# kvcache-ai/ktransformers

Measured on NVIDIA H100. Metric: decode tok/s DeepSeek-V3 671B INT4 (Q4_K_M) MoE-block hot path; HBM GB/s vs roofline, higher is better.
Workload: dtype int8xint4/int6->int32 dp4a, fp32 scales+accumulate, bf16 in/out

## Files before the change

### ktransformers_b200/csrc/handles.cuh

```cuda
#pragma once
#include "common.cuh"

namespace ktb {
enum FmtId { FMT_Q4K, FMT_Q5K, FMT_Q6K8, FMT_Q6K4T, FMT_GENK, FMT_RAWINT4, FMT_NONE };
enum Q6Layout { LAYOUT_RAW = 0, LAYOUT_SOA8 = 1, LAYOUT_T4 = 2 };

static inline FmtId pick_fmt(int type, int layout) {
    if (type == KTB200_TYPE_Q4_K) return FMT_Q4K;
    if (type == KTB200_TYPE_Q5_K) return FMT_Q5K;
    if (type == KTB200_TYPE_Q6_K && layout == LAYOUT_SOA8) return FMT_Q6K8;
    if (type == KTB200_TYPE_Q6_K && layout == LAYOUT_T4) return FMT_Q6K4T;
    if (is_kquant(type) || is_iquant(type)) return FMT_GENK;
    if (is_rawint4(type)) return FMT_RAWINT4;
    return FMT_NONE;
}
}

struct ktb200_mlp {
    int H, I, gate_type, up_type, down_type, hidden_type, group_max_len, device;
    const void *gate, *up, *down;
    bool loaded, gu_soa;
    int down_layout;
    float* inter;
};
// ... 1 lines not shown
struct ktb200_moe {
    ktb200_moe_config cfg;
    int device;
    bool loaded;
    bool gu_soa;
    int down_layout;
    float* inter;
    int64_t* ids_d;
    float* w_d;
    void* in_d;
    void* out_d;
    float* blk_partial;
    unsigned* blk_sync;
    unsigned blk_flip;
    float* blk_inter;
    uint8_t* blk_stage;
    const void* pf[3];
    size_t pf_bytes[3];
};

namespace ktb {
constexpr int kBlockMaxTokens = 8;
constexpr int kBlkStatusWord = 4, kBlkReadyWord = 8;
static inline size_t blk_ready_words(const ktb200_moe_config& c) {
    const int t = c.group_max_len < kBlockMaxTokens ? c.group_max_len : kBlockMaxTokens;
    return (size_t)t * (c.routed_expert_num + 1) * (c.intermediate_size / QK_K);
}
}

struct DeviceGuard {
    int prev;
    bool ok;
    explicit DeviceGuard(int dev) : prev(0), ok(true) {
        if (cudaGetDevice(&prev) != cudaSuccess) ok = false;
        if (ok && prev != dev && cudaSetDevice(dev) != cudaSuccess) ok = false;
    }
    ~DeviceGuard() { cudaSetDevice(prev); }
};
```

### ktransformers_b200/csrc/moe.cu

```cuda
#include <cstdio>
#include <cstdlib>
#include <cstring>
#include <new>

#define KTB_IQ_CODEBOOKS
#include "gemv_bulk.cuh"
#include "dense_bulk.cuh"
#include "rawint4.cuh"
#include "iq.cuh"
#include "handles.cuh"

namespace ktb {

__global__ void __launch_bounds__(256) repack_q6k_kernel(uint8_t* w, long n_groups, int nb) {
    extern __shared__ __align__(16) uint8_t smem[];
    const long gbytes = 8L * SZ_Q6_K * nb;
    for (long g = blockIdx.x; g < n_groups; g += gridDim.x) {
        uint8_t* base = w + g * gbytes;
        for (long i = threadIdx.x; i < gbytes / 16; i += blockDim.x)
            reinterpret_cast<uint4*>(smem)[i] = reinterpret_cast<const uint4*>(base)[i];
        __syncthreads();
        const uint16_t* src = reinterpret_cast<const uint16_t*>(smem);
        uint16_t* dst = reinterpret_cast<uint16_t*>(base);
        const long s_qh = 1024L * nb, s_sc = 1536L * nb, s_d = 1664L * nb;
// ... 559 lines not shown
        set_error("MOEConfig: hidden_size %d and intermediate_size %d must be multiples of 256 for K-quant tensors",
                  c->hidden_size, c->intermediate_size);
        return KTB200_EINVAL;
    }
    if (!c->gate_proj || !c->up_proj || !c->down_proj) { set_error("MOEConfig: null weight pointer"); return KTB200_EINVAL; }
    DeviceGuard g(device);
    if (!g.ok) { set_error("cudaSetDevice(%d) failed", device); return KTB200_ECUDA; }
    ktb200_moe* m = new (std::nothrow) ktb200_moe();
    if (!m) return KTB200_ENOMEM;
    m->cfg = *c;
    m->device = device;
    m->loaded = false;
    m->gu_soa = false;
    m->down_layout = LAYOUT_RAW;
    m->inter = nullptr; m->ids_d = nullptr; m->w_d = nullptr; m->in_d = nullptr; m->out_d = nullptr;
    m->blk_partial = nullptr; m->blk_sync = nullptr; m->blk_flip = 0; m->blk_inter = nullptr; m->blk_stage = nullptr;
    for (int r = 0; r < 3; r++) { m->pf[r] = nullptr; m->pf_bytes[r] = 0; }
    const size_t slots = (size_t)c->group_max_len * c->routed_expert_num;
    const size_t hid = (size_t)c->group_max_len * c->hidden_size * type_size(c->hidden_type);
    cudaError_t e = cudaMalloc(&m->inter, (slots + c->group_max_len) * c->intermediate_size * sizeof(float));
    if (e == cudaSuccess) e = cudaMalloc(&m->ids_d, slots * sizeof(int64_t));
    if (e == cudaSuccess) e = cudaMalloc(&m->w_d, slots * sizeof(float));
    if (e == cudaSuccess) e = cudaMalloc(&m->in_d, hid);
    if (e == cudaSuccess) e = cudaMalloc(&m->out_d, hid);
    if (e == cudaSuccess) e = cudaMalloc(&m->blk_partial, (size_t)8 * 8 * 512 * sizeof(float));
    const size_t sync_words = kBlkReadyWord + 2 * blk_ready_words(*c);
    if (e == cudaSuccess) e = cudaMalloc(&m->blk_sync, sync_words * sizeof(unsigned));
    if (e == cudaSuccess) e = cudaMemset(m->blk_sync, 0, sync_words * sizeof(unsigned));
    if (e == cudaSuccess) e = cudaMalloc(&m->blk_inter, blk_ready_words(*c) * QK_K * sizeof(float));
    if (e == cudaSuccess) e = cudaMemset(m->blk_inter, 0xff, blk_ready_words(*c) * QK_K * sizeof(float));
    if (e == cudaSuccess) e = cudaMalloc(&m->blk_stage, blk_ready_words(*c) * (QK_K + 32 + 4));
    if (e != cudaSuccess) {
        set_error("cudaMalloc failed: %s", cudaGetErrorString(e));
        ktb200_moe_destroy(m);
        return KTB200_ENOMEM;
    }
    *out = m;
    return KTB200_OK;
}

void ktb200_moe_destroy(ktb200_moe* m) {
    if (!m) return;
    DeviceGuard g(m->device);
    cudaFree(m->inter); cudaFree(m->ids_d); cudaFree(m->w_d); cudaFree(m->in_d); cudaFree(m->out_d);
    cudaFree(m->blk_partial); cudaFree(m->blk_sync); cudaFree(m->blk_inter); cudaFree(m->blk_stage);
    delete m;
}

int ktb200_moe_load_weights(ktb200_moe* m, void* stream) {
    if (!m) { set_error("null handle"); return KTB200_EINVAL; }
    if (m->loaded) return KTB200_OK;
    DeviceGuard g(m->device);
    const ktb200_moe_config& c = m->cfg;
    cudaStream_t s = (cudaStream_t)stream;
    if (c.gate_type == KTB200_TYPE_Q6_K && c.up_type == KTB200_TYPE_Q6_K && c.intermediate_size % 8 == 0) {
        int rc = repack_q6k(const_cast<void*>(c.gate_proj), (long)c.expert_num * c.intermediate_size, c.hidden_size, m->device, s);
        if (rc) return rc;
        rc = repack_q6k(const_cast<void*>(c.up_proj), (long)c.expert_num * c.intermediate_size, c.hidden_size, m->device, s);
        if (rc) return rc;
        m->gu_soa = true;
// ... 341 lines not shown
```

### ktransformers_b200/csrc/moe_block.cu

```cuda
#include <cstdlib>

#include "gate.cuh"
#include "gemv_bulk.cuh"
#include "handles.cuh"

namespace ktb {

constexpr int kBlockWarps = 15;
constexpr int kBlockWarpsLo = 12;

struct BlockParams {
    GateParams g;
    const void *w_gate, *w_up, *w_down;
    const void *s_gate, *s_up, *s_down;
    int n_local, id_offset;
    int H, I, k;
    int hidden_type, use_silu;
    float* inter;
    void* out;
    unsigned* sync;
    unsigned* ready;
    unsigned* status;
    uint8_t* stage_q;
    int16_t* stage_bs;
    float* stage_d;
    int nrows_max;
    int region_a;
    int ring_bytes;
    int prime_u, prime_d;
    unsigned long long* trace;
    const uint8_t* pf[3];
    unsigned pf_bytes[3];
};

__device__ __forceinline__ unsigned ld_acquire_u32(const unsigned* p) {
    unsigned v;
    asm volatile("ld.acquire.gpu.global.u32 %0, [%1];" : "=r"(v) : "l"(p) : "memory");
    return v;
}
__device__ __forceinline__ unsigned ld_acquire_sys_u32(const unsigned* p) {
// ... 31 lines not shown
__device__ __forceinline__ void grid_wait(unsigned* counter, unsigned gen) {
    if (threadIdx.x == 0) {
        const unsigned target = gen * gridDim.x;
        while (ld_acquire_u32(counter) < target) {}
    }
    __syncthreads();
}


__device__ __forceinline__ void trace_stamp(const BlockParams& p, int i) {
    if (p.trace) p.trace[blockIdx.x * 16 + i] = ep_now();
}
__device__ __forceinline__ void block_stamp(const BlockParams& p, int i) {
    if (threadIdx.x == 0) trace_stamp(p, i);
}

__device__ __forceinline__ float4 load_x4(const void* x, long i4, int type) {
    if (type == KTB200_TYPE_F32) return reinterpret_cast<const float4*>(x)[i4];
    const uint2 v = reinterpret_cast<const uint2*>(x)[i4];
    if (type == KTB200_TYPE_BF16)
        return make_float4(__uint_as_float(v.x << 16), __uint_as_float(v.x & 0xffff0000u), __uint_as_float(v.y << 16),
                           __uint_as_float(v.y & 0xffff0000u));
    const float2 a = __half22float2(*reinterpret_cast<const __half2*>(&v.x)), b = __half22float2(*reinterpret_cast<const __half2*>(&v.y));
    return make_float4(a.x, a.y, b.x, b.y);
}

struct BlockShared {
    BlockParams prm;
    int64_t ids[32];
    float w[32];
    int vs[36];
    int nv;
    unsigned skip;
    int ent_state[36];
    int last_cta;
};
constexpr int kBlockSharedBytes = (sizeof(BlockShared) + 15) & ~15;

struct BlockLay {
    uint8_t *xq, *aq;
    int16_t *xbs, *abs_;
    float *xdx, *adx, *sel, *partial;
    size_t ring_off;
};
template <int KBS>
__device__ __forceinline__ BlockLay block_layout(const BlockParams& p, uint8_t* smem) {
    const int nblk = p.H / QK_K, nb = p.I / QK_K, ns = p.k + (p.s_gate ? 1 : 0);
    uint8_t* a = smem + kBlockSharedBytes;
    BlockLay L;
// ... 87 lines not shown
        int nv = p.s_gate ? 1 : 0;
        for (int j = 0; j < k; j++) {
            const long e = (long)sh.ids[j] - p.id_offset;
            if (e < 0 || e >= p.n_local) sk |= 1u << j; else sh.vs[nv++] = j;
        }
        sh.nv = nv;
        sh.skip = sk;
    }
    if (blockIdx.x == 0 && threadIdx.x < k) {
        p.g.idx[(long)t * k + threadIdx.x] = sh.ids[threadIdx.x];
        p.g.w[(long)t * k + threadIdx.x] = sh.w[threadIdx.x];
    }
    __syncthreads();
}

__device__ __forceinline__ void entry_slice(int I, int ie, int& r0, int& len) {
    const unsigned s = (blockIdx.x + (unsigned)ie) % gridDim.x;
    r0 = (int)((unsigned long long)I * s / gridDim.x);
    len = (int)((unsigned long long)I * (s + 1) / gridDim.x) - r0;
}

constexpr unsigned kInterEmpty = 0xffffffffu;
__device__ __forceinline__ void st_relaxed_f32(float* p, float v) {
    asm volatile("st.relaxed.gpu.global.f32 [%0], %1;" ::"l"(p), "f"(v) : "memory");
}
__device__ __forceinline__ uint4 ld_relaxed_u4(const void* p) {
    uint4 v;
    asm volatile("ld.relaxed.gpu.global.v4.u32 {%0, %1, %2, %3}, [%4];" : "=r"(v.x), "=r"(v.y), "=r"(v.z), "=r"(v.w) : "l"(p) : "memory");
    return v;
}

template <int KBS>
__device__ __forceinline__ void quantise_block(const BlockParams& p, long gb, float* src) {
    const int lane = threadIdx.x & 31;
    uint4 v0, v1;
    unsigned long long t0 = 0;
    for (unsigned spins = 1;; spins++) {
        v0 = ld_relaxed_u4(src + lane * 8);
        v1 = ld_relaxed_u4(src + lane * 8 + 4);
        const bool here = v0.x != kInterEmpty && v0.y != kInterEmpty && v0.z != kInterEmpty && v0.w != kInterEmpty &&
                          v1.x != kInterEmpty && v1.y != kInterEmpty && v1.z != kInterEmpty && v1.w != kInterEmpty;
        if (__all_sync(0xffffffffu, here)) break;
        if ((spins & 255u) == 0) {
            const unsigned long long t = ep_now();
            if (!t0) t0 = t;
            else if (t - t0 > kEpTimeoutNs) { if (lane == 0) *p.status = 1; break; }
        }
    }
    const float x[8] = {__uint_as_float(v0.x), __uint_as_float(v0.y), __uint_as_float(v0.z), __uint_as_float(v0.w),
                        __uint_as_float(v1.x), __uint_as_float(v1.y), __uint_as_float(v1.z), __uint_as_float(v1.w)};
    warp_quantize_q8k_block(x, lane, reinterpret_cast<uint32_t*>(p.stage_q + gb * QK_K), p.stage_d + gb,
                            KBS == 16 ? p.stage_bs + gb * 16 : nullptr, KBS == 8 ? p.stage_bs + gb * 8 : nullptr);
    const uint4 empty = make_uint4(kInterEmpty, kInterEmpty, kInterEmpty, kInterEmpty);
    reinterpret_cast<uint4*>(src + lane * 8)[0] = empty;
    reinterpret_cast<uint4*>(src + lane * 8)[1] = empty;
    __syncwarp();
    if (lane == 0) {
        __threadfence();
        atomicExch(p.ready + gb, 2u);
    }
}

template <int KBS>
__device__ __forceinline__ void claim_entry(const BlockParams& p, int t, int slot) {
    const int lane = threadIdx.x & 31, ns = p.k + (p.s_gate ? 1 : 0), nb = p.I / QK_K;
    const long g0 = ((long)t * ns + slot) * nb;
    for (int c0 = 0; c0 < nb; c0 += 32) {
        const int nc = min(32, nb - c0), rot = (int)(blockIdx.x % nc);
        for (;;) {
            const unsigned fr = __ballot_sync(0xffffffffu, lane < nc && ld_acquire_u32(p.ready + g0 + c0 + lane) == 0u);
            if (!fr) break;
            const unsigned pref = fr & (~0u << rot);
            const int b = c0 + __ffs(pref ? pref : fr) - 1;
            unsigned won = 0;
            if (lane == 0) won = atomicCAS(p.ready + g0 + b, 0u, 1u) == 0u;
            if (__shfl_sync(0xffffffffu, won, 0)) quantise_block<KBS>(p, g0 + b, p.inter + ((long)t * ns + slot) * p.I + (long)b * QK_K);
        }
    }
}

template <int KBS>
__device__ __forceinline__ void entry_to_smem(BlockShared& sh, const BlockLay& L, int t, int ev, bool need) {
    const BlockParams& p = sh.prm;
    const int lane = threadIdx.x & 31;
    volatile int* state = &sh.ent_state[ev];
    int s = lane == 0 ? *state : 0;
    s = __shfl_sync(0xffffffffu, s, 0);
    if (s == 0) {
        if (lane == 0) s = atomicCAS(&sh.ent_state[ev], 0, 1) == 0 ? 3 : 1;
        s = __shfl_sync(0xffffffffu, s, 0);
    }
    if (s == 3) {
        const int nb = p.I / QK_K, slot = sh.vs[ev];
        const long g0 = ((long)t * (p.k + (p.s_gate ? 1 : 0)) + slot) * nb;
        for (int b = lane; b < nb; b += 32) wait_ge<false>(p.ready + g0 + b, 2u, p.status);
        __syncwarp();
        const uint4* q = reinterpret_cast<const uint4*>(p.stage_q + g0 * QK_K);
        for (int i = lane; i < nb * (QK_K / 16); i += 32)
            *reinterpret_cast<uint4*>(L.aq + (size_t)(slot * nb + i / (QK_K / 16)) * kActBlkStride + (i % (QK_K / 16)) * 16) = __ldcg(q + i);
        const uint4* bs = reinterpret_cast<const uint4*>(p.stage_bs + g0 * KBS);
        for (int i = lane; i < nb * KBS / 8; i += 32) reinterpret_cast<uint4*>(L.abs_ + slot * nb * KBS)[i] = __ldcg(bs + i);
        for (int i = lane; i < nb; i += 32) L.adx[slot * nb + i] = __ldcg(p.stage_d + g0 + i);
        __syncwarp();
        if (lane == 0) {
            __threadfence_block();
            *state = 2;
            if (ev == 0) trace_stamp(p, 6);
            if (ev == sh.nv - 1) trace_stamp(p, 7);
        }
    } else if (s == 1 && need && lane == 0) {
        while (*state != 2) {}
    }
    if (lane == 0) __threadfence_block();
    __syncwarp();
}

template <int KBS>
__device__ __forceinline__ void blk_combine(int t) {
    extern __shared__ __align__(16) uint8_t smem[];
    const BlockShared& sh = *reinterpret_cast<const BlockShared*>(smem);
    const BlockParams& p = sh.prm;
    const BlockLay L = block_layout<KBS>(p, smem);
    const int k = p.k, ns = k + (p.s_gate ? 1 : 0);
    const int quads = p.H / 4;
    const int q0 = (int)((long)quads * blockIdx.x / gridDim.x), nrows = ((int)((long)quads * (blockIdx.x + 1) / gridDim.x) - q0) * 4;
    const unsigned skip = sh.skip;
// ... 30 lines not shown
    if (lane == 0) {
#pragma unroll
        for (int s = 0; s < SU; s++) mbar_init(bar_u32 + 8 * s, 1);
        mbar_fence_init();
        fence_proxy_async_smem();
    }
    {
        const uint32_t* src = reinterpret_cast<const uint32_t*>(&p);
        uint32_t* dst = reinterpret_cast<uint32_t*>(&sh.prm);
        for (int i = threadIdx.x; i < (int)(sizeof(BlockParams) / 4); i += blockDim.x) dst[i] = src[i];
    }
    if (threadIdx.x == 0 && has_shared) sh.vs[0] = k;
    uint32_t phase = 0;
    unsigned gen = 0;
    block_stamp(p, 0);

  for (int t = 0; t < Teff; t++) {
    __syncthreads();
    {
        const int nblk = p.H / QK_K, row_bytes = nblk * SZ_Q4_K;
        const int ns = k + (has_shared ? 1 : 0);
        int ie = 0, ir = 0, ir0 = 0, ilen = 0, ileft = 0, isub = 0;
        int ce = 0, cr = 0, cr0 = 0, clen = 0, cleft = 0, csub = 0;
        int stride = W, iend = 1;
        int slot_i = 0, slot_u = 0;
        auto advance = [&](int& e, int& r, int& r0, int& len, int n) {
            int off = r - r0 + n;
            while (off >= len && e + 1 < iend) { off -= len; e++; entry_slice(p.I, e, r0, len); }
            r = r0 + off;
        };
        auto start_list = [&](int e0, int e1, int first, int count, int stride_) {
            iend = e1;
            ie = e0;
            entry_slice(p.I, e0, ir0, ilen);
            ir = ir0;
            advance(ie, ir, ir0, ilen, first);
            ce = ie; cr = ir; cr0 = ir0; clen = ilen;
            ileft = cleft = count > 0 ? count : 0;
            stride = stride_;
        };
        auto issue_u = [&]() {
            if (ileft > 0 && isub - csub < SU) {
                if (lane == 0) {
                    const int s = sh.vs[ie];
                    const bool second = isub & 1;
                    const uint8_t* src;
                    if (s == k) {
                        src = reinterpret_cast<const uint8_t*>(second ? p.s_up : p.s_gate) + (long)ir * row_bytes;
                    } else {
                        const long e = (long)sh.ids[s] - p.id_offset;
                        src = reinterpret_cast<const uint8_t*>(second ? p.w_up : p.w_gate) + (e * p.I + ir) * row_bytes;
                    }
                    const uint32_t bar = bar_u32 + 8 * slot_i;
                    mbar_expect_tx(bar, (uint32_t)row_bytes);
                    bulk_g2s(ring_u32 + slot_i * row_bytes, src, (uint32_t)row_bytes, bar);
                }
                isub++;
                if (!(isub & 1)) {
                    ileft--;
                    advance(ie, ir, ir0, ilen, stride);
                }
                slot_i = (slot_i + 1 == SU) ? 0 : slot_i + 1;
            }
        };
        if (threadIdx.x < 36) sh.ent_state[threadIdx.x] = 0;
        blk_router(t, waited);
        block_stamp(p, 2);
        grid_arrive(p.sync, gen);
        if (has_shared && warp >= kGateWarps) {
            int r0, nr;
            entry_slice(p.I, 0, r0, nr);
            const int first = warp - kGateWarps, st = W - kGateWarps;
            start_list(0, 1, first, (nr - first + st - 1) / st, st);
        }
#pragma unroll
        for (int s = 0; s < SU; s++)
            if (s < p.prime_u) issue_u();
        blk_quantize_x(t);
        block_stamp(p, 1);
        grid_wait(p.sync, gen);
        block_stamp(p, 3);
        const BlockLay L = block_layout<DownFmt::kBs>(p, smem);
        const uint8_t* ring = smem + (ring_u32 - (uint32_t)__cvta_generic_to_shared(smem));
#pragma unroll 1
        for (int list = 0; list < 2; list++) {
            if (list == 1) {
                blk_select(t);
                block_stamp(p, 4);
                const int e0 = has_shared ? 1 : 0, nv = sh.nv;
                int total = 0;
                for (int e = e0; e < nv; e++) {
                    int r0, len;
                    entry_slice(p.I, e, r0, len);
                    total += len;
                }
                start_list(e0, nv, warp, (total - warp + W - 1) / W, W);
#pragma unroll
                for (int s = 0; s < SU; s++) issue_u();
            }
            float acc_first = 0.f;
            while (cleft > 0) {
                mbar_wait(bar_u32 + 8 * slot_u, (phase >> slot_u) & 1u);
                phase ^= 1u << slot_u;
                const uint8_t* row0 = ring + slot_u * row_bytes;
                float acc = 0.f;
                if (lane < nblk)
                    acc = q4k_block_dot(row0 + lane * SZ_Q4_K, L.xq + (size_t)lane * kActBlkStride,
                                        *reinterpret_cast<const uint4*>(L.xbs + lane * 8), L.xdx[lane]);
                __syncwarp();
                slot_u = (slot_u + 1 == SU) ? 0 : slot_u + 1;
                csub++;
                issue_u();
                if (csub & 1) { acc_first = acc; continue; }
                float g = acc_first, uu = acc;
#pragma unroll
                for (int o = 16; o > 0; o >>= 1) {
                    g += __shfl_xor_sync(0xffffffffu, g, o);
                    uu += __shfl_xor_sync(0xffffffffu, uu, o);
                }
                if (lane == 0) st_relaxed_f32(p.inter + ((long)t * ns + sh.vs[ce]) * p.I + cr, (p.use_silu ? act_silu(g) : act_relu(g)) * uu);
                cleft--;
                advance(ce, cr, cr0, clen, stride);
            }
        }
        __syncthreads();
        block_stamp(p, 5);
    }
    {
        const int nb = p.I / QK_K, nrb = RW * nb, item_bytes = nrb * DownFmt::kBlockBytes;
        const int quads = p.H / RW;
        const int q0 = (int)((long)quads * blockIdx.x / gridDim.x), nquads = (int)((long)quads * (blockIdx.x + 1) / gridDim.x) - q0;
        const int nv = sh.nv;
        const int Wd = W - 1;
        int ni = warp < Wd ? nquads * nv - warp : 0;
        ni = ni > 0 ? (ni + Wd - 1) / Wd : 0;
        int dvi = 0, dq = 0, dss = 0, dcons = 0;
        if (ni > 0) { dvi = warp / nquads; dq = warp - dvi * nquads; }
        int evi = dvi, eq = dq;
        int dslot_i = 0, dslot_u = 0;
        auto issue_d = [&]() {
            if (dss < ni && dss - dcons < SD) {
                if (lane == 0) {
                    const int j = sh.vs[dvi];
                    long row = (long)(q0 + dq) * RW;
                    const uint8_t* wbase = reinterpret_cast<const uint8_t*>(p.w_down);
                    if (j == k) wbase = reinterpret_cast<const uint8_t*>(p.s_down);
                    else row += ((long)sh.ids[j] - p.id_offset) * p.H;
                    const uint32_t bar = bar_u32 + 8 * dslot_i;
                    mbar_expect_tx(bar, (uint32_t)item_bytes);
                    bulk_g2s(ring_u32 + dslot_i * item_bytes, wbase + (row >> 2) * item_bytes, (uint32_t)item_bytes, bar);
                }
                dss++;
                dq += Wd;
                while (dq >= nquads) { dq -= nquads; dvi++; }
                dslot_i = (dslot_i + 1 == SD) ? 0 : dslot_i + 1;
            }
        };
#pragma unroll
        for (int s = 0; s < SD; s++) issue_d();
        const BlockLay L = block_layout<DownFmt::kBs>(p, smem);
        if (warp == W - 1) {
            for (int ev = 0; ev < nv; ev++) claim_entry<DownFmt::kBs>(p, t, sh.vs[ev]);
        }
        if (t == Teff - 1 && warp == W - 1) {
#pragma unroll
            for (int r = 0; r < 3; r++) {
                if (p.pf[r]) {
                    const unsigned per = ((p.pf_bytes[r] / gridDim.x) + 15u) & ~15u;
                    const unsigned lo = per * blockIdx.x, hi = min(p.pf_bytes[r], lo + per);
                    for (unsigned o = lo + lane * 4096u; o < hi; o += 32u * 4096u) prefetch_l2_bulk(p.pf[r] + o, min(4096u, hi - o) & ~15u);
                }
            }
        }

        const uint8_t* ring = smem + (ring_u32 - (uint32_t)__cvta_generic_to_shared(smem));
        const int ns = k + (has_shared ? 1 : 0);
        for (int n = 0; n < ni; n++) {
            if (eq < Wd) {
                entry_to_smem<DownFmt::kBs>(sh, L, t, evi, true);
                if (evi + 1 < nv) entry_to_smem<DownFmt::kBs>(sh, L, t, evi + 1, false);
            }
            mbar_wait(bar_u32 + 8 * dslot_u, (phase >> dslot_u) & 1u);
            phase ^= 1u << dslot_u;
            const uint8_t* sl = ring + dslot_u * item_bytes;
            const int j = sh.vs[evi];
            float res;
            {
                float acc[RW] = {0.f, 0.f, 0.f, 0.f};
                for (int f = lane; f < nrb; f += 32) {
                    const int rw = f / nb, blk = f - rw * nb;
                    const int ab = j * nb + blk;
                    const float val = DownFmt::dot(sl, f, nrb, L.aq + (size_t)ab * kActBlkStride, L.abs_ + ab * DownFmt::kBs, L.adx[ab]);
                    acc[0] += rw == 0 ? val : 0.f; acc[1] += rw == 1 ? val : 0.f; acc[2] += rw == 2 ? val : 0.f; acc[3] += rw == 3 ? val : 0.f;
                }
                res = warp_reduce4(acc[0], acc[1], acc[2], acc[3], lane);
            }
            __syncwarp();
            dslot_u = (dslot_u + 1 == SD) ? 0 : dslot_u + 1;
            dcons++;
            issue_d();
            if ((lane & 7) == 0) L.partial[(eq * RW + (lane >> 3)) * ns + j] = res;
            eq += Wd;
            while (eq >= nquads) { eq -= nquads; evi++; }
        }
        __syncthreads();
        block_stamp(p, 8);
        blk_combine<DownFmt::kBs>(t);
        block_stamp(p, 9);
    }
  }

    __syncthreads();
    if (threadIdx.x == 0) sh.last_cta = atomicAdd(p.sync + 1, 1u) == gridDim.x - 1;
    __syncthreads();
    if (sh.last_cta) {
        const int nready = Teff * (k + (has_shared ? 1 : 0)) * (p.I / QK_K);
        for (int i = threadIdx.x; i < nready; i += blockDim.x) p.ready[i] = 0;
        if (threadIdx.x == 0) {
            p.sync[0] = 0;
            p.sync[1] = 0;
        }
        __threadfence();
    }
}


constexpr int kEpWorldMax = 8;
constexpr int kEpPairsMax = 64;

struct EpExtra {
    int rank, world, phase_mask, pa;
    int msg_bytes;
// ... 453 lines not shown
        if (rc) return rc;
        return ktb200_moe_forward_shared(m, sh, qlen, k, idx, w, input, output, bsz, stream);
    }

    const int S = gate_splits(gc->n_experts, gc->hidden_size, num_sms(dev));
    p.g = GateParams{gc->weight, input, gc->hidden_type, gc->n_experts, gc->hidden_size, qlen, S, k, gc->n_group, gc->topk_group,
                     gc->scoring, gc->topk_method, gc->norm_topk_prob, gc->routed_scaling_factor, gc->bias, m->blk_partial, nullptr,
                     idx, w, bsz, nullptr};
    p.w_gate = c.gate_proj; p.w_up = c.up_proj; p.w_down = c.down_proj;
    p.s_gate = sh ? sh->gate : nullptr; p.s_up = sh ? sh->up : nullptr; p.s_down = sh ? sh->down : nullptr;
    p.n_local = c.expert_num; p.id_offset = c.expert_id_offset;
    p.H = c.hidden_size; p.I = c.intermediate_size; p.k = k; p.hidden_type = c.hidden_type; p.use_silu = c.use_silu;
    const unsigned flip = m->blk_flip++ & 1u;
    p.inter = m->blk_inter; p.out = output; p.sync = m->blk_sync + 2 * flip; p.trace = g_btrace;
    p.status = m->blk_sync + kBlkStatusWord;
    p.ready = m->blk_sync + kBlkReadyWord + flip * blk_ready_words(c);
    p.stage_q = m->blk_stage;
    p.stage_bs = reinterpret_cast<int16_t*>(m->blk_stage + blk_ready_words(c) * (size_t)QK_K);
    p.stage_d = reinterpret_cast<float*>(m->blk_stage + blk_ready_words(c) * (size_t)(QK_K + 32));
    for (int r = 0; r < 3; r++) { p.pf[r] = (const uint8_t*)m->pf[r]; p.pf_bytes[r] = (unsigned)m->pf_bytes[r]; }
    static const int prime_u = [] { const char* e = getenv("KTB200_BLK_PRIME_U"); return e ? atoi(e) : 3; }();
    p.prime_u = prime_u;

    void* args[] = {&p};
    const void* fn;
    if (W > kBlockWarpsLo) fn = fd == FMT_Q6K4T ? (const void*)moe_block_kernel<BulkQ6K4T, kBlockWarps> : (const void*)moe_block_kernel<BulkQ4K, kBlockWarps>;
    else fn = fd == FMT_Q6K4T ? (const void*)moe_block_kernel<BulkQ6K4T, kBlockWarpsLo> : (const void*)moe_block_kernel<BulkQ4K, kBlockWarpsLo>;
    static const int coop = [] { const char* e = getenv("KTB200_BLK_COOP"); return e ? atoi(e) : 1; }();
    static const int pdl = [] { const char* e = getenv("KTB200_BLK_PDL"); return e ? atoi(e) : 1; }();
    auto separate = [&]() -> int {
        int rc = ktb200_moe_gate_forward(gc, qlen, input, idx, w, nullptr, bsz, stream);
        if (rc) return rc;
        return ktb200_moe_forward_shared(m, sh, qlen, k, idx, w, input, output, bsz, stream);
    };
// ... 173 lines not shown
    if (cudaPointerGetAttributes(&pa, output) == cudaSuccess && pa.type == cudaMemoryTypeHost && pa.devicePointer) out_dev = pa.devicePointer;
    else (void)cudaGetLastError();
    int rc = ktb200_moe_block_forward(gc, m, sh, qlen, m->in_d, out_dev, m->ids_d, m->w_d, nullptr, stream);
    if (rc) return rc;
    if (out_dev == m->out_d) KTB_CUDA_CHECK(cudaMemcpyAsync(output, m->out_d, hid, cudaMemcpyDeviceToHost, s));
    if (idx) KTB_CUDA_CHECK(cudaMemcpyAsync(idx, m->ids_d, (size_t)qlen * k * sizeof(int64_t), cudaMemcpyDeviceToHost, s));
    if (w) KTB_CUDA_CHECK(cudaMemcpyAsync(w, m->w_d, (size_t)qlen * k * sizeof(float), cudaMemcpyDeviceToHost, s));
    KTB_CUDA_CHECK(cudaStreamSynchronize(s));
    return KTB200_OK;
}

extern "C" void ktb200_debug_block_trace(unsigned long long* trace_dev) { g_btrace = trace_dev; }

extern "C" long ktb200_debug_block_sync_words(ktb200_moe* m, unsigned* host_out, long n) {
    if (!m) { set_error("null handle"); return -1; }
    const long total = (long)(kBlkReadyWord + 2 * blk_ready_words(m->cfg));
    DeviceGuard guard(m->device);
    if (host_out && n > 0) {
        if (cudaDeviceSynchronize() != cudaSuccess ||
            cudaMemcpy(host_out, m->blk_sync, (size_t)(n < total ? n : total) * sizeof(unsigned), cudaMemcpyDeviceToHost) != cudaSuccess) {
            set_error("debug_block_sync_words: %s", cudaGetErrorString(cudaGetLastError()));
            return -1;
        }
    }
    return total;
}
```

### profiles/block_trace.py

```python
#!/usr/bin/env python
import ctypes as C
import os
import sys

sys.path.insert(0, os.path.dirname(os.path.dirname(os.path.abspath(__file__))))
import numpy as np
import torch

from ktransformers_b200 import native
from ktransformers_b200.util.synth import synth_blocks

lib = native.lib()
E, K, H, I = 256, 8, 7168, 2048
Q4_K, Q6_K, BF16 = 12, 14, 30
S = lambda: torch.cuda.current_stream().cuda_stream
layers = []
for l in range(3):
    g, u, d = synth_blocks(Q4_K, E * I * H, device="cuda", seed=3 * l), synth_blocks(Q4_K, E * I * H, device="cuda", seed=3 * l + 1), synth_blocks(Q6_K, E * H * I, device="cuda", seed=3 * l + 2)
    sg, su, sd = synth_blocks(Q4_K, I * H, device="cuda", seed=100 + l), synth_blocks(Q4_K, I * H, device="cuda", seed=200 + l), synth_blocks(Q6_K, H * I, device="cuda", seed=300 + l)
    cfg = native.MoeConfig(E, K, H, I, 64, 10, 8, 1, g.data_ptr(), u.data_ptr(), d.data_ptr(), Q4_K, Q4_K, Q6_K, BF16, 0)
    moe = C.c_void_p(); native.check(lib.ktb200_moe_create(C.byref(cfg), 0, C.byref(moe))); native.check(lib.ktb200_moe_load_weights(moe, S()))
    mlp = C.c_void_p(); native.check(lib.ktb200_mlp_create(H, I, sg.data_ptr(), su.data_ptr(), sd.data_ptr(), Q4_K, Q4_K, Q6_K, BF16, 8, 0, C.byref(mlp)))
    native.check(lib.ktb200_mlp_load_weights(mlp, S()))
    W = torch.randn(E, H, device="cuda"); b = torch.randn(E, device="cuda")
    gc = native.GateConfig(E, H, K, 8, 4, 0, 0, 1, 2.5, W.data_ptr(), b.data_ptr(), BF16)
    layers.append((gc, moe, mlp, (g, u, d, sg, su, sd, W, b)))
x = (torch.randn(1, H, device="cuda") / 100).to(torch.bfloat16)
y = torch.zeros(1, H, dtype=torch.bfloat16, device="cuda")
ids = torch.zeros(1, K, dtype=torch.int64, device="cuda"); wts = torch.zeros(1, K, device="cuda")
n_sm = torch.cuda.get_device_properties(torch.cuda.current_device()).multi_processor_count
trace = torch.zeros(n_sm * 16, dtype=torch.int64, device="cuda")
names = ["start", "x quantised (under barrier 1)", "router partials written", "grid barrier 1 passed", "top-k selected",
         "gate/up done (CTA)", "entry 0 ready (its a in smem)", "last entry ready (its a in smem)", "down tiles done (CTA)", "combined + stored",
         "  (top-k done, before the work-list build)"]
acc = []
for rep in range(12):
    gc, moe, mlp, _ = layers[rep % 3]
    lib.ktb200_debug_block_trace(trace.data_ptr())
    native.check(lib.ktb200_moe_block_forward(C.byref(gc), moe, mlp, 1, x.data_ptr(), y.data_ptr(), ids.data_ptr(), wts.data_ptr(), None, S()))
    torch.cuda.synchronize()
    t = trace.cpu().numpy().reshape(n_sm, 16)[:, :11].astype(np.float64)
    t -= t[:, 0].min()
    if rep >= 3:
        acc.append(t)
lib.ktb200_debug_block_trace(None)
t = np.mean(acc, axis=0) / 1e3
print(f"{'boundary':42s} {'first':>8s} {'median':>8s} {'last':>8s}   (us after the first CTA started; mean of {len(acc)} launches)")
for i in sorted(range(len(names)), key=lambda i: np.median(t[:, i])):
    print(f"{names[i]:42s} {t[:, i].min():8.2f} {np.median(t[:, i]):8.2f} {t[:, i].max():8.2f}")
```

Before: 160.2.

## Use dynamic work-stealing for routed gate/up rows and quantise activations per CTA

Static per-entry row slicing of routed gate/up work is replaced by a global atomic unit counter, so warps claim rows dynamically and slow SMs no longer hold back the grid. The cross-CTA quantise/stage handshake (ready flags, global staging buffers, CAS claims) is dropped. Each CTA now quantises the intermediate activations directly into shared memory, claiming blocks through per-entry shared counters. This removes global staging traffic and the ready-flag protocol, but every CTA now repeats the quantisation work, and the atomic counter plus per-row destination bookkeeping add overhead. The down-phase warp count also changes from Wd to W, and tracing gains an SM id stamp.

```diff
diff --git a/ktransformers_b200/csrc/handles.cuh b/ktransformers_b200/csrc/handles.cuh
--- a/ktransformers_b200/csrc/handles.cuh
+++ b/ktransformers_b200/csrc/handles.cuh
@@ -39,17 +39,16 @@
     unsigned* blk_sync;
     unsigned blk_flip;
     float* blk_inter;
-    uint8_t* blk_stage;
     const void* pf[3];
     size_t pf_bytes[3];
 };
 
 namespace ktb {
 constexpr int kBlockMaxTokens = 8;
-constexpr int kBlkStatusWord = 4, kBlkReadyWord = 8;
-static inline size_t blk_ready_words(const ktb200_moe_config& c) {
+constexpr int kBlkStatusWord = 4, kBlkUnitWord = 8, kBlkSyncWords = kBlkUnitWord + 2 * kBlockMaxTokens;
+static inline size_t blk_inter_floats(const ktb200_moe_config& c) {
     const int t = c.group_max_len < kBlockMaxTokens ? c.group_max_len : kBlockMaxTokens;
-    return (size_t)t * (c.routed_expert_num + 1) * (c.intermediate_size / QK_K);
+    return (size_t)t * (c.routed_expert_num + 1) * c.intermediate_size;
 }
 }
 
diff --git a/ktransformers_b200/csrc/moe.cu b/ktransformers_b200/csrc/moe.cu
--- a/ktransformers_b200/csrc/moe.cu
+++ b/ktransformers_b200/csrc/moe.cu
@@ -597,7 +597,7 @@
     m->gu_soa = false;
     m->down_layout = LAYOUT_RAW;
     m->inter = nullptr; m->ids_d = nullptr; m->w_d = nullptr; m->in_d = nullptr; m->out_d = nullptr;
-    m->blk_partial = nullptr; m->blk_sync = nullptr; m->blk_flip = 0; m->blk_inter = nullptr; m->blk_stage = nullptr;
+    m->blk_partial = nullptr; m->blk_sync = nullptr; m->blk_flip = 0; m->blk_inter = nullptr;
     for (int r = 0; r < 3; r++) { m->pf[r] = nullptr; m->pf_bytes[r] = 0; }
     const size_t slots = (size_t)c->group_max_len * c->routed_expert_num;
     const size_t hid = (size_t)c->group_max_len * c->hidden_size * type_size(c->hidden_type);
@@ -607,12 +607,10 @@
     if (e == cudaSuccess) e = cudaMalloc(&m->in_d, hid);
     if (e == cudaSuccess) e = cudaMalloc(&m->out_d, hid);
     if (e == cudaSuccess) e = cudaMalloc(&m->blk_partial, (size_t)8 * 8 * 512 * sizeof(float));
-    const size_t sync_words = kBlkReadyWord + 2 * blk_ready_words(*c);
-    if (e == cudaSuccess) e = cudaMalloc(&m->blk_sync, sync_words * sizeof(unsigned));
-    if (e == cudaSuccess) e = cudaMemset(m->blk_sync, 0, sync_words * sizeof(unsigned));
-    if (e == cudaSuccess) e = cudaMalloc(&m->blk_inter, blk_ready_words(*c) * QK_K * sizeof(float));
-    if (e == cudaSuccess) e = cudaMemset(m->blk_inter, 0xff, blk_ready_words(*c) * QK_K * sizeof(float));
-    if (e == cudaSuccess) e = cudaMalloc(&m->blk_stage, blk_ready_words(*c) * (QK_K + 32 + 4));
+    if (e == cudaSuccess) e = cudaMalloc(&m->blk_sync, kBlkSyncWords * sizeof(unsigned));
+    if (e == cudaSuccess) e = cudaMemset(m->blk_sync, 0, kBlkSyncWords * sizeof(unsigned));
+    if (e == cudaSuccess) e = cudaMalloc(&m->blk_inter, blk_inter_floats(*c) * sizeof(float));
+    if (e == cudaSuccess) e = cudaMemset(m->blk_inter, 0xff, blk_inter_floats(*c) * sizeof(float));
     if (e != cudaSuccess) {
         set_error("cudaMalloc failed: %s", cudaGetErrorString(e));
         ktb200_moe_destroy(m);
@@ -626,7 +624,7 @@
     if (!m) return;
     DeviceGuard g(m->device);
     cudaFree(m->inter); cudaFree(m->ids_d); cudaFree(m->w_d); cudaFree(m->in_d); cudaFree(m->out_d);
-    cudaFree(m->blk_partial); cudaFree(m->blk_sync); cudaFree(m->blk_inter); cudaFree(m->blk_stage);
+    cudaFree(m->blk_partial); cudaFree(m->blk_sync); cudaFree(m->blk_inter);
     delete m;
 }
 
diff --git a/ktransformers_b200/csrc/moe_block.cu b/ktransformers_b200/csrc/moe_block.cu
--- a/ktransformers_b200/csrc/moe_block.cu
+++ b/ktransformers_b200/csrc/moe_block.cu
@@ -19,11 +19,8 @@
     float* inter;
     void* out;
     unsigned* sync;
-    unsigned* ready;
+    unsigned* units;
     unsigned* status;
-    uint8_t* stage_q;
-    int16_t* stage_bs;
-    float* stage_d;
     int nrows_max;
     int region_a;
     int ring_bytes;
@@ -85,6 +82,13 @@
 __device__ __forceinline__ void block_stamp(const BlockParams& p, int i) {
     if (threadIdx.x == 0) trace_stamp(p, i);
 }
+__device__ __forceinline__ void trace_smid(const BlockParams& p) {
+    if (p.trace && threadIdx.x == 0) {
+        unsigned sm;
+        asm volatile("mov.u32 %0, %%smid;" : "=r"(sm));
+        p.trace[blockIdx.x * 16 + 12] = sm;
+    }
+}
 
 __device__ __forceinline__ float4 load_x4(const void* x, long i4, int type) {
     if (type == KTB200_TYPE_F32) return reinterpret_cast<const float4*>(x)[i4];
@@ -103,7 +107,9 @@
     int vs[36];
     int nv;
     unsigned skip;
-    int ent_state[36];
+    int ent_claim[36];
+    int ent_done[36];
+    int udst[kBlockWarps][4];
     int last_cta;
 };
 constexpr int kBlockSharedBytes = (sizeof(BlockShared) + 15) & ~15;
@@ -221,12 +227,6 @@
     __syncthreads();
 }
 
-__device__ __forceinline__ void entry_slice(int I, int ie, int& r0, int& len) {
-    const unsigned s = (blockIdx.x + (unsigned)ie) % gridDim.x;
-    r0 = (int)((unsigned long long)I * s / gridDim.x);
-    len = (int)((unsigned long long)I * (s + 1) / gridDim.x) - r0;
-}
-
 constexpr unsigned kInterEmpty = 0xffffffffu;
 __device__ __forceinline__ void st_relaxed_f32(float* p, float v) {
     asm volatile("st.relaxed.gpu.global.f32 [%0], %1;" ::"l"(p), "f"(v) : "memory");
@@ -238,85 +238,48 @@
 }
 
 template <int KBS>
-__device__ __forceinline__ void quantise_block(const BlockParams& p, long gb, float* src) {
-    const int lane = threadIdx.x & 31;
-    uint4 v0, v1;
-    unsigned long long t0 = 0;
-    for (unsigned spins = 1;; spins++) {
-        v0 = ld_relaxed_u4(src + lane * 8);
-        v1 = ld_relaxed_u4(src + lane * 8 + 4);
-        const bool here = v0.x != kInterEmpty && v0.y != kInterEmpty && v0.z != kInterEmpty && v0.w != kInterEmpty &&
-                          v1.x != kInterEmpty && v1.y != kInterEmpty && v1.z != kInterEmpty && v1.w != kInterEmpty;
-        if (__all_sync(0xffffffffu, here)) break;
-        if ((spins & 255u) == 0) {
-            const unsigned long long t = ep_now();
-            if (!t0) t0 = t;
-            else if (t - t0 > kEpTimeoutNs) { if (lane == 0) *p.status = 1; break; }
-        }
-    }
-    const float x[8] = {__uint_as_float(v0.x), __uint_as_float(v0.y), __uint_as_float(v0.z), __uint_as_float(v0.w),
-                        __uint_as_float(v1.x), __uint_as_float(v1.y), __uint_as_float(v1.z), __uint_as_float(v1.w)};
-    warp_quantize_q8k_block(x, lane, reinterpret_cast<uint32_t*>(p.stage_q + gb * QK_K), p.stage_d + gb,
-                            KBS == 16 ? p.stage_bs + gb * 16 : nullptr, KBS == 8 ? p.stage_bs + gb * 8 : nullptr);
-    const uint4 empty = make_uint4(kInterEmpty, kInterEmpty, kInterEmpty, kInterEmpty);
-    reinterpret_cast<uint4*>(src + lane * 8)[0] = empty;
-    reinterpret_cast<uint4*>(src + lane * 8)[1] = empty;
-    __syncwarp();
-    if (lane == 0) {
-        __threadfence();
-        atomicExch(p.ready + gb, 2u);
-    }
-}
-
-template <int KBS>
-__device__ __forceinline__ void claim_entry(const BlockParams& p, int t, int slot) {
-    const int lane = threadIdx.x & 31, ns = p.k + (p.s_gate ? 1 : 0), nb = p.I / QK_K;
-    const long g0 = ((long)t * ns + slot) * nb;
-    for (int c0 = 0; c0 < nb; c0 += 32) {
-        const int nc = min(32, nb - c0), rot = (int)(blockIdx.x % nc);
-        for (;;) {
-            const unsigned fr = __ballot_sync(0xffffffffu, lane < nc && ld_acquire_u32(p.ready + g0 + c0 + lane) == 0u);
-            if (!fr) break;
-            const unsigned pref = fr & (~0u << rot);
-            const int b = c0 + __ffs(pref ? pref : fr) - 1;
-            unsigned won = 0;
-            if (lane == 0) won = atomicCAS(p.ready + g0 + b, 0u, 1u) == 0u;
-            if (__shfl_sync(0xffffffffu, won, 0)) quantise_block<KBS>(p, g0 + b, p.inter + ((long)t * ns + slot) * p.I + (long)b * QK_K);
-        }
-    }
-}
-
-template <int KBS>
 __device__ __forceinline__ void entry_to_smem(BlockShared& sh, const BlockLay& L, int t, int ev, bool need) {
     const BlockParams& p = sh.prm;
-    const int lane = threadIdx.x & 31;
-    volatile int* state = &sh.ent_state[ev];
-    int s = lane == 0 ? *state : 0;
-    s = __shfl_sync(0xffffffffu, s, 0);
-    if (s == 0) {
-        if (lane == 0) s = atomicCAS(&sh.ent_state[ev], 0, 1) == 0 ? 3 : 1;
-        s = __shfl_sync(0xffffffffu, s, 0);
-    }
-    if (s == 3) {
-        const int nb = p.I / QK_K, slot = sh.vs[ev];
-        const long g0 = ((long)t * (p.k + (p.s_gate ? 1 : 0)) + slot) * nb;
-        for (int b = lane; b < nb; b += 32) wait_ge<false>(p.ready + g0 + b, 2u, p.status);
-        __syncwarp();
-        const uint4* q = reinterpret_cast<const uint4*>(p.stage_q + g0 * QK_K);
-        for (int i = lane; i < nb * (QK_K / 16); i += 32)
-            *reinterpret_cast<uint4*>(L.aq + (size_t)(slot * nb + i / (QK_K / 16)) * kActBlkStride + (i % (QK_K / 16)) * 16) = __ldcg(q + i);
-        const uint4* bs = reinterpret_cast<const uint4*>(p.stage_bs + g0 * KBS);
-        for (int i = lane; i < nb * KBS / 8; i += 32) reinterpret_cast<uint4*>(L.abs_ + slot * nb * KBS)[i] = __ldcg(bs + i);
-        for (int i = lane; i < nb; i += 32) L.adx[slot * nb + i] = __ldcg(p.stage_d + g0 + i);
+    const int lane = threadIdx.x & 31, nb = p.I / QK_K, slot = sh.vs[ev];
+    const float* src0 = p.inter + ((long)t * (p.k + (p.s_gate ? 1 : 0)) + slot) * p.I;
+    for (;;) {
+        int b = 0;
+        if (lane == 0) b = atomicAdd(&sh.ent_claim[ev], 1);
+        b = __shfl_sync(0xffffffffu, b, 0);
+        if (b >= nb) break;
+        const float* src = src0 + (long)b * QK_K;
+        uint4 v0, v1;
+        unsigned long long t0 = 0;
+        for (unsigned spins = 1;; spins++) {
+            v0 = ld_relaxed_u4(src + lane * 8);
+            v1 = ld_relaxed_u4(src + lane * 8 + 4);
+            const bool here = v0.x != kInterEmpty && v0.y != kInterEmpty && v0.z != kInterEmpty && v0.w != kInterEmpty &&
+                              v1.x != kInterEmpty && v1.y != kInterEmpty && v1.z != kInterEmpty && v1.w != kInterEmpty;
+            if (__all_sync(0xffffffffu, here)) break;
+            if ((spins & 255u) == 0) {
+                const unsigned long long tn = ep_now();
+                if (!t0) t0 = tn;
+                else if (tn - t0 > kEpTimeoutNs) { if (lane == 0) *p.status = 1; break; }
+            }
+        }
+        const float x[8] = {__uint_as_float(v0.x), __uint_as_float(v0.y), __uint_as_float(v0.z), __uint_as_float(v0.w),
+                            __uint_as_float(v1.x), __uint_as_float(v1.y), __uint_as_float(v1.z), __uint_as_float(v1.w)};
+        const int ab = slot * nb + b;
+        warp_quantize_q8k_block(x, lane, reinterpret_cast<uint32_t*>(L.aq + (size_t)ab * kActBlkStride), L.adx + ab,
+                                KBS == 16 ? L.abs_ + ab * 16 : nullptr, KBS == 8 ? L.abs_ + ab * 8 : nullptr);
         __syncwarp();
         if (lane == 0) {
             __threadfence_block();
-            *state = 2;
-            if (ev == 0) trace_stamp(p, 6);
-            if (ev == sh.nv - 1) trace_stamp(p, 7);
-        }
-    } else if (s == 1 && need && lane == 0) {
-        while (*state != 2) {}
+            if (atomicAdd(&sh.ent_done[ev], 1) == nb - 1) {
+                if (ev == 0) trace_stamp(p, 6);
+                if (ev == sh.nv - 1) trace_stamp(p, 7);
+            }
+        }
+        if (!need) break;
+    }
+    if (need && lane == 0) {
+        const volatile int* done = &sh.ent_done[ev];
+        while (*done < nb) {}
     }
     if (lane == 0) __threadfence_block();
     __syncwarp();
@@ -377,64 +340,58 @@
     uint32_t phase = 0;
     unsigned gen = 0;
     block_stamp(p, 0);
+    trace_smid(p);
 
   for (int t = 0; t < Teff; t++) {
     __syncthreads();
     {
         const int nblk = p.H / QK_K, row_bytes = nblk * SZ_Q4_K;
-        const int ns = k + (has_shared ? 1 : 0);
-        int ie = 0, ir = 0, ir0 = 0, ilen = 0, ileft = 0, isub = 0;
-        int ce = 0, cr = 0, cr0 = 0, clen = 0, cleft = 0, csub = 0;
-        int stride = W, iend = 1;
+        const int ns = k + (has_shared ? 1 : 0), e0 = has_shared ? 1 : 0;
+        int iu = 0, iend = 0, istep = 0;
+        bool routed = false;
+        unsigned nxt = 0;
+        int isub = 0, csub = 0;
         int slot_i = 0, slot_u = 0;
-        auto advance = [&](int& e, int& r, int& r0, int& len, int n) {
-            int off = r - r0 + n;
-            while (off >= len && e + 1 < iend) { off -= len; e++; entry_slice(p.I, e, r0, len); }
-            r = r0 + off;
-        };
-        auto start_list = [&](int e0, int e1, int first, int count, int stride_) {
-            iend = e1;
-            ie = e0;
-            entry_slice(p.I, e0, ir0, ilen);
-            ir = ir0;
-            advance(ie, ir, ir0, ilen, first);
-            ce = ie; cr = ir; cr0 = ir0; clen = ilen;
-            ileft = cleft = count > 0 ? count : 0;
-            stride = stride_;
-        };
         auto issue_u = [&]() {
-            if (ileft > 0 && isub - csub < SU) {
+            if (iu < iend && isub - csub < SU) {
+                const bool second = isub & 1;
                 if (lane == 0) {
-                    const int s = sh.vs[ie];
-                    const bool second = isub & 1;
                     const uint8_t* src;
-                    if (s == k) {
-                        src = reinterpret_cast<const uint8_t*>(second ? p.s_up : p.s_gate) + (long)ir * row_bytes;
+                    int s = k, row = iu;
+                    if (routed) {
+                        const int e = e0 + iu / p.I;
+                        row = iu - (e - e0) * p.I;
+                        s = sh.vs[e];
+                        const long ex = (long)sh.ids[s] - p.id_offset;
+                        src = reinterpret_cast<const uint8_t*>(second ? p.w_up : p.w_gate) + (ex * p.I + row) * row_bytes;
                     } else {
-                        const long e = (long)sh.ids[s] - p.id_offset;
-                        src = reinterpret_cast<const uint8_t*>(second ? p.w_up : p.w_gate) + (e * p.I + ir) * row_bytes;
+                        src = reinterpret_cast<const uint8_t*>(second ? p.s_up : p.s_gate) + (long)row * row_bytes;
                     }
+                    if (second) sh.udst[warp][slot_i] = (t * ns + s) * p.I + row;
                     const uint32_t bar = bar_u32 + 8 * slot_i;
                     mbar_expect_tx(bar, (uint32_t)row_bytes);
                     bulk_g2s(ring_u32 + slot_i * row_bytes, src, (uint32_t)row_bytes, bar);
                 }
                 isub++;
-                if (!(isub & 1)) {
-                    ileft--;
-                    advance(ie, ir, ir0, ilen, stride);
+                if (second) {
+                    if (routed) {
+                        iu = (int)__shfl_sync(0xffffffffu, nxt, 0);
+                        if (lane == 0 && iu < iend) nxt = atomicAdd(p.units + t, 1u);
+                    } else {
+                        iu += istep;
+                    }
                 }
                 slot_i = (slot_i + 1 == SU) ? 0 : slot_i + 1;
             }
         };
-        if (threadIdx.x < 36) sh.ent_state[threadIdx.x] = 0;
+        if (threadIdx.x < 36) { sh.ent_claim[threadIdx.x] = 0; sh.ent_done[threadIdx.x] = 0; }
         blk_router(t, waited);
         block_stamp(p, 2);
         grid_arrive(p.sync, gen);
         if (has_shared && warp >= kGateWarps) {
-            int r0, nr;
-            entry_slice(p.I, 0, r0, nr);
-            const int first = warp - kGateWarps, st = W - kGateWarps;
-            start_list(0, 1, first, (nr - first + st - 1) / st, st);
+            iu = (int)((long)p.I * blockIdx.x / gridDim.x) + warp - kGateWarps;
+            iend = (int)((long)p.I * (blockIdx.x + 1) / gridDim.x);
+            istep = W - kGateWarps;
         }
 #pragma unroll
         for (int s = 0; s < SU; s++)
@@ -443,6 +400,11 @@
         block_stamp(p, 1);
         grid_wait(p.sync, gen);
         block_stamp(p, 3);
+        unsigned first_u = 0;
+        if (lane == 0) {
+            first_u = atomicAdd(p.units + t, 2u);
+            nxt = first_u + 1;
+        }
         const BlockLay L = block_layout<DownFmt::kBs>(p, smem);
         const uint8_t* ring = smem + (ring_u32 - (uint32_t)__cvta_generic_to_shared(smem));
 #pragma unroll 1
@@ -450,21 +412,17 @@
             if (list == 1) {
                 blk_select(t);
                 block_stamp(p, 4);
-                const int e0 = has_shared ? 1 : 0, nv = sh.nv;
-                int total = 0;
-                for (int e = e0; e < nv; e++) {
-                    int r0, len;
-                    entry_slice(p.I, e, r0, len);
-                    total += len;
-                }
-                start_list(e0, nv, warp, (total - warp + W - 1) / W, W);
+                routed = true;
+                iu = (int)__shfl_sync(0xffffffffu, first_u, 0);
+                iend = (sh.nv - e0) * p.I;
 #pragma unroll
                 for (int s = 0; s < SU; s++) issue_u();
             }
             float acc_first = 0.f;
-            while (cleft > 0) {
+            while (csub < isub) {
                 mbar_wait(bar_u32 + 8 * slot_u, (phase >> slot_u) & 1u);
                 phase ^= 1u << slot_u;
+                const int dst = lane == 0 ? sh.udst[warp][slot_u] : 0;
                 const uint8_t* row0 = ring + slot_u * row_bytes;
                 float acc = 0.f;
                 if (lane < nblk)
@@ -481,9 +439,7 @@
                     g += __shfl_xor_sync(0xffffffffu, g, o);
                     uu += __shfl_xor_sync(0xffffffffu, uu, o);
                 }
-                if (lane == 0) st_relaxed_f32(p.inter + ((long)t * ns + sh.vs[ce]) * p.I + cr, (p.use_silu ? act_silu(g) : act_relu(g)) * uu);
-                cleft--;
-                advance(ce, cr, cr0, clen, stride);
+                if (lane == 0) st_relaxed_f32(p.inter + dst, (p.use_silu ? act_silu(g) : act_relu(g)) * uu);
             }
         }
         __syncthreads();
@@ -494,9 +450,8 @@
         const int quads = p.H / RW;
         const int q0 = (int)((long)quads * blockIdx.x / gridDim.x), nquads = (int)((long)quads * (blockIdx.x + 1) / gridDim.x) - q0;
         const int nv = sh.nv;
-        const int Wd = W - 1;
-        int ni = warp < Wd ? nquads * nv - warp : 0;
-        ni = ni > 0 ? (ni + Wd - 1) / Wd : 0;
+        int ni = nquads * nv - warp;
+        ni = ni > 0 ? (ni + W - 1) / W : 0;
         int dvi = 0, dq = 0, dss = 0, dcons = 0;
         if (ni > 0) { dvi = warp / nquads; dq = warp - dvi * nquads; }
         int evi = dvi, eq = dq;
@@ -514,7 +469,7 @@
                     bulk_g2s(ring_u32 + dslot_i * item_bytes, wbase + (row >> 2) * item_bytes, (uint32_t)item_bytes, bar);
                 }
                 dss++;
-                dq += Wd;
+                dq += W;
                 while (dq >= nquads) { dq -= nquads; dvi++; }
                 dslot_i = (dslot_i + 1 == SD) ? 0 : dslot_i + 1;
             }
@@ -522,9 +477,6 @@
 #pragma unroll
         for (int s = 0; s < SD; s++) issue_d();
         const BlockLay L = block_layout<DownFmt::kBs>(p, smem);
-        if (warp == W - 1) {
-            for (int ev = 0; ev < nv; ev++) claim_entry<DownFmt::kBs>(p, t, sh.vs[ev]);
-        }
         if (t == Teff - 1 && warp == W - 1) {
 #pragma unroll
             for (int r = 0; r < 3; r++) {
@@ -539,12 +491,13 @@
         const uint8_t* ring = smem + (ring_u32 - (uint32_t)__cvta_generic_to_shared(smem));
         const int ns = k + (has_shared ? 1 : 0);
         for (int n = 0; n < ni; n++) {
-            if (eq < Wd) {
+            if (eq < W) {
                 entry_to_smem<DownFmt::kBs>(sh, L, t, evi, true);
                 if (evi + 1 < nv) entry_to_smem<DownFmt::kBs>(sh, L, t, evi + 1, false);
             }
             mbar_wait(bar_u32 + 8 * dslot_u, (phase >> dslot_u) & 1u);
             phase ^= 1u << dslot_u;
+            if (n == 0 && warp == 0 && lane == 0) trace_stamp(p, 11);
             const uint8_t* sl = ring + dslot_u * item_bytes;
             const int j = sh.vs[evi];
             float res;
@@ -563,7 +516,7 @@
             dcons++;
             issue_d();
             if ((lane & 7) == 0) L.partial[(eq * RW + (lane >> 3)) * ns + j] = res;
-            eq += Wd;
+            eq += W;
             while (eq >= nquads) { eq -= nquads; evi++; }
         }
         __syncthreads();
@@ -577,8 +530,10 @@
     if (threadIdx.x == 0) sh.last_cta = atomicAdd(p.sync + 1, 1u) == gridDim.x - 1;
     __syncthreads();
     if (sh.last_cta) {
-        const int nready = Teff * (k + (has_shared ? 1 : 0)) * (p.I / QK_K);
-        for (int i = threadIdx.x; i < nready; i += blockDim.x) p.ready[i] = 0;
+        const int ninter = Teff * (k + (has_shared ? 1 : 0)) * p.I / 4;
+        const uint4 empty = make_uint4(kInterEmpty, kInterEmpty, kInterEmpty, kInterEmpty);
+        for (int i = threadIdx.x; i < ninter; i += blockDim.x) reinterpret_cast<uint4*>(p.inter)[i] = empty;
+        if ((int)threadIdx.x < Teff) p.units[threadIdx.x] = 0;
         if (threadIdx.x == 0) {
             p.sync[0] = 0;
             p.sync[1] = 0;
@@ -1062,10 +1017,7 @@
     const unsigned flip = m->blk_flip++ & 1u;
     p.inter = m->blk_inter; p.out = output; p.sync = m->blk_sync + 2 * flip; p.trace = g_btrace;
     p.status = m->blk_sync + kBlkStatusWord;
-    p.ready = m->blk_sync + kBlkReadyWord + flip * blk_ready_words(c);
-    p.stage_q = m->blk_stage;
-    p.stage_bs = reinterpret_cast<int16_t*>(m->blk_stage + blk_ready_words(c) * (size_t)QK_K);
-    p.stage_d = reinterpret_cast<float*>(m->blk_stage + blk_ready_words(c) * (size_t)(QK_K + 32));
+    p.units = m->blk_sync + kBlkUnitWord + flip * kBlockMaxTokens;
     for (int r = 0; r < 3; r++) { p.pf[r] = (const uint8_t*)m->pf[r]; p.pf_bytes[r] = (unsigned)m->pf_bytes[r]; }
     static const int prime_u = [] { const char* e = getenv("KTB200_BLK_PRIME_U"); return e ? atoi(e) : 3; }();
     p.prime_u = prime_u;
@@ -1269,7 +1221,7 @@
 
 extern "C" long ktb200_debug_block_sync_words(ktb200_moe* m, unsigned* host_out, long n) {
     if (!m) { set_error("null handle"); return -1; }
-    const long total = (long)(kBlkReadyWord + 2 * blk_ready_words(m->cfg));
+    const long total = kBlkSyncWords;
     DeviceGuard guard(m->device);
     if (host_out && n > 0) {
         if (cudaDeviceSynchronize() != cudaSuccess ||
diff --git a/profiles/block_trace.py b/profiles/block_trace.py
--- a/profiles/block_trace.py
+++ b/profiles/block_trace.py
@@ -1,7 +1,16 @@
 #!/usr/bin/env python
+import argparse
 import ctypes as C
 import os
 import sys
+
+ap = argparse.ArgumentParser()
+ap.add_argument("--graph", action="store_true")
+ap.add_argument("--chain", type=int, default=12, help="--graph: launches captured back to back")
+ap.add_argument("--replays", type=int, default=10, help="--graph: timed replays of the chain")
+args = ap.parse_args()
+if args.graph:
+    os.environ.setdefault("KTB200_BLK_COOP", "0")
 
 sys.path.insert(0, os.path.dirname(os.path.dirname(os.path.abspath(__file__))))
 import numpy as np
@@ -29,22 +38,81 @@
 y = torch.zeros(1, H, dtype=torch.bfloat16, device="cuda")
 ids = torch.zeros(1, K, dtype=torch.int64, device="cuda"); wts = torch.zeros(1, K, device="cuda")
 n_sm = torch.cuda.get_device_properties(torch.cuda.current_device()).multi_processor_count
-trace = torch.zeros(n_sm * 16, dtype=torch.int64, device="cuda")
 names = ["start", "x quantised (under barrier 1)", "router partials written", "grid barrier 1 passed", "top-k selected",
          "gate/up done (CTA)", "entry 0 ready (its a in smem)", "last entry ready (its a in smem)", "down tiles done (CTA)", "combined + stored",
-         "  (top-k done, before the work-list build)"]
-acc = []
-for rep in range(12):
+         "  (top-k done, before the work-list build)", "first down tile consumed (warp 0)"]
+NT = len(names)
+
+
+def launch(rep, trace_ptr):
     gc, moe, mlp, _ = layers[rep % 3]
-    lib.ktb200_debug_block_trace(trace.data_ptr())
+    lib.ktb200_debug_block_trace(trace_ptr)
     native.check(lib.ktb200_moe_block_forward(C.byref(gc), moe, mlp, 1, x.data_ptr(), y.data_ptr(), ids.data_ptr(), wts.data_ptr(), None, S()))
+
+
+runs = []
+if not args.graph:
+    trace = torch.zeros(n_sm * 16, dtype=torch.int64, device="cuda")
+    for rep in range(12):
+        launch(rep, trace.data_ptr())
+        torch.cuda.synchronize()
+        if rep >= 3:
+            runs.append(trace.cpu().numpy().reshape(n_sm, 16).copy())
+else:
+    n = args.chain
+    trace = torch.zeros(n, n_sm * 16, dtype=torch.int64, device="cuda")
+    for rep in range(3 * n):
+        launch(rep, trace[rep % n].data_ptr())
     torch.cuda.synchronize()
-    t = trace.cpu().numpy().reshape(n_sm, 16)[:, :11].astype(np.float64)
-    t -= t[:, 0].min()
-    if rep >= 3:
-        acc.append(t)
+    side = torch.cuda.Stream()
+    side.wait_stream(torch.cuda.current_stream())
+    graph = torch.cuda.CUDAGraph()
+    with torch.cuda.graph(graph, stream=side):
+        for rep in range(n):
+            launch(rep, trace[rep].data_ptr())
+    for r in range(args.replays + 1):
+        trace.zero_()
+        graph.replay()
+        torch.cuda.synchronize()
+        if r == 0:
+            continue
+        tr = trace.cpu().numpy().reshape(n, n_sm, 16)
+        for rep in range(1, n):
+            runs.append(tr[rep].copy())
 lib.ktb200_debug_block_trace(None)
-t = np.mean(acc, axis=0) / 1e3
-print(f"{'boundary':42s} {'first':>8s} {'median':>8s} {'last':>8s}   (us after the first CTA started; mean of {len(acc)} launches)")
-for i in sorted(range(len(names)), key=lambda i: np.median(t[:, i])):
-    print(f"{names[i]:42s} {t[:, i].min():8.2f} {np.median(t[:, i]):8.2f} {t[:, i].max():8.2f}")
+
+stats = []
+for tr in runs:
+    t = tr[:, :NT].astype(np.float64)
+    t = (t - t[:, 0].min()) / 1e3
+    stats.append(np.stack([t.min(0), np.median(t, 0), t.max(0)], 1))
+st = np.mean(stats, axis=0)
+mode = f"captured chains of {args.chain}, {args.replays} replays, plain grid + PDL" if args.graph else "isolated launches"
+print(f"{'boundary':42s} {'first':>8s} {'median':>8s} {'last':>8s}   (us after the launch's first CTA started; mean over "
+      f"{len(runs)} launches, {mode})")
+for i in sorted(range(NT), key=lambda i: st[i, 1]):
+    print(f"{names[i]:42s} {st[i, 0]:8.2f} {st[i, 1]:8.2f} {st[i, 2]:8.2f}")
+
+print()
+per = {"gate/up: top-k selected -> gate/up done": (4, 5), "wait: gate/up done -> first down tile consumed": (5, 11),
+       "down: first down tile consumed -> down tiles done": (11, 8), "down: gate/up done -> down tiles done": (5, 8)}
+print(f"{'per-CTA duration (us)':52s} {'min':>7s} {'median':>7s} {'max':>7s}")
+for name, (a, b) in per.items():
+    d = np.array([np.percentile((tr[:, b] - tr[:, a]) / 1e3, [0, 50, 100]) for tr in runs]).mean(0)
+    print(f"{name:52s} {d[0]:7.2f} {d[1]:7.2f} {d[2]:7.2f}")
+if args.graph:
+    ends = np.array([tr[:, 9].max() for tr in runs], dtype=np.float64).reshape(args.replays, args.chain - 1)
+    print(f"\nlaunch period in the chain (last CTA done -> next launch's last CTA done): {np.diff(ends, axis=1).mean() / 1e3:.2f} us")
+
+sm_done = np.full((len(runs), n_sm), np.nan)
+for i, tr in enumerate(runs):
+    sm_done[i, tr[:, 12].astype(np.int64)] = (tr[:, 5] - tr[:, 0].min()) / 1e3
+slow = max(1, n_sm // 10)
+sets = [set(np.argsort(r)[-slow:].tolist()) for r in sm_done]
+overlap = np.mean([len(sets[i] & sets[i + 1]) / slow for i in range(len(sets) - 1)]) if len(sets) > 1 else float("nan")
+rk = np.argsort(np.argsort(sm_done, axis=1), axis=1).astype(np.float64)
+corr = np.mean([np.corrcoef(rk[i], rk[i + 1])[0, 1] for i in range(len(rk) - 1)]) if len(rk) > 1 else float("nan")
+freq = np.bincount(np.concatenate([list(s) for s in sets]), minlength=n_sm)
+print(f"\nslowest {slow} SMs at 'gate/up done': {overlap:.2f} of them are again among the slowest in the next launch "
+      f"(chance: {slow / n_sm:.2f}); rank correlation between consecutive launches {corr:.2f}")
+print("SMs most often among the slowest:", ", ".join(f"{s} ({freq[s]}/{len(sets)})" for s in np.argsort(freq)[::-1][:8]))
```

After: 161.9, median of 6. +1.0%, better.
